# werner-duvaud/muzero-general

Hardware: NVIDIA H100
Metric: self-play env-steps/sec (higher is better)
Workload: dtype f32 nets + f64 tree statistics

## Files before the change

### muzero_general_b200/csrc/fc_search.cu

```cuda
#include "fc_net.cuh"
#include "tree.cuh"
#include "kernels.h"

#include <stdlib.h>
#include <algorithm>
#include <vector>

namespace mz {

struct GameSmem {
    int vsum, mval, root_prior, visit, expansion, reward, prior, path, path_reward, hidden, act, bytes;
};

__host__ __device__ inline GameSmem game_smem_layout(int N, int A, int E, int maxw, bool keep_hidden) {
    GameSmem L;
    const int S = (N + 1) * A;
    const int Epad = (E + 3) & ~3;
    int off = 0;
    auto take = [&](int bytes) { int o = off; off = (off + bytes + 15) & ~15; return o; };
    L.vsum = take(S * 8);
    L.mval = take(S * 8);
    L.root_prior = take(A * 8);
    L.visit = take(S * 4);
    L.expansion = take(S * 4);
    L.reward = take(S * 4);
    L.prior = take(S * 4);
    L.path = take((N + 2) * 4);
    L.path_reward = take((N + 2) * 4);
    L.hidden = take((keep_hidden ? (N + 1) * Epad : 0) * 4);
    L.act = take(9 * maxw * 4);
    off += 16;
    L.bytes = off;
    return L;
}

enum { kPhRoot, kPhSelect, kPhNet, kPhExpand, kPhBackup, kPhLevels, kPhRounds, kPhSims, kPhSums,
       kPhStart = kPhSums, kPhEnd, kPhCount };
#ifdef MZ_FC_PHASES
constexpr int kPhMaxGames = 1 << 16;
__device__ unsigned long long g_fc_phase[kPhMaxGames][kPhCount];
MZ_DEVINL unsigned long long global_ns() {
    unsigned long long t;
    asm volatile("mov.u64 %0, %%globaltimer;" : "=l"(t));
    return t;
}
struct PhaseClock {
    int row = -1;
    unsigned last = 0;
    MZ_DEVINL void start(int g, bool leader) {
        row = (leader && g < kPhMaxGames) ? g : -1;
        if (row >= 0) atomicExch(&g_fc_phase[row][kPhStart], global_ns());
        last = (unsigned)clock();
    }
    MZ_DEVINL void finish() { if (row >= 0) atomicExch(&g_fc_phase[row][kPhEnd], global_ns()); }
    MZ_DEVINL void mark(int p) {
        const unsigned now = (unsigned)clock();
        if (row >= 0) atomicAdd(&g_fc_phase[row][p], (unsigned long long)(now - last));
        last = now;
    }
    MZ_DEVINL void count(int p, int n) { if (row >= 0) atomicAdd(&g_fc_phase[row][p], (unsigned long long)n); }
};
#else
struct PhaseClock {
    MZ_DEVINL void start(int, bool) {}
    MZ_DEVINL void finish() {}
    MZ_DEVINL void mark(int) {}
    MZ_DEVINL void count(int, int) {}
};
#endif

template <typename SH>
constexpr int fixed_actions() {
    if constexpr (SH::kEnabled) return SH::A;
    else return 0;
}

template <int G, bool kTeacher, typename SH, int kP>
__global__ void __launch_bounds__(kFcMaxThreads, 2) fc_search_kernel(const __grid_constant__ FcSearchArgs a) {
    extern __shared__ __align__(16) unsigned char smem[];
    constexpr int kA = fixed_actions<SH>();
    const int N = a.N, A = kA ? kA : a.A;
    double* s_pbc = reinterpret_cast<double*>(smem);
    double* s_sqrt = s_pbc + (N + 2);
    float* s_blob = reinterpret_cast<float*>(s_sqrt + (N + 2));
    for (int i = threadIdx.x; i < N + 2; i += blockDim.x) { s_pbc[i] = a.pbc[i]; s_sqrt[i] = a.sqrtn[i]; }
    if (!kTeacher)
        for (int i = threadIdx.x; i < a.net.blob_floats; i += blockDim.x) s_blob[i] = a.blob[i];
    __syncthreads();

    const int shared_bytes = ((2 * (N + 2) * 8 + (kTeacher ? 0 : a.net.blob_floats) * 4) + 15) & ~15;
    const GameSmem L = game_smem_layout(N, A, a.net.E, a.net.maxw, !kTeacher);
    const int groups_per_cta = blockDim.x / G;
    const int gi = threadIdx.x / G;
    const int lane = LaneGroup<G>::lane();
    unsigned char* mine = smem + shared_bytes + (size_t)gi * L.bytes;

    TreeConst c;
    c.A = A; c.N = N; c.P = a.P; c.discount = a.discount; c.noise_frac = a.noise_frac; c.noise_alpha = a.noise_alpha; c.seed = a.seed;
    c.pbc = s_pbc; c.sqrtn = s_sqrt; c.ucb = a.ucb;

    GameTree t;
    t.vsum = reinterpret_cast<double*>(mine + L.vsum);
    t.mval = reinterpret_cast<double*>(mine + L.mval);
    t.root_prior = reinterpret_cast<double*>(mine + L.root_prior);
    t.visit = reinterpret_cast<int*>(mine + L.visit);
    t.expansion = reinterpret_cast<int*>(mine + L.expansion);
    t.reward = reinterpret_cast<float*>(mine + L.reward);
    t.prior = reinterpret_cast<float*>(mine + L.prior);
    t.path = reinterpret_cast<int*>(mine + L.path);
    t.path_reward = reinterpret_cast<float*>(mine + L.path_reward);
    float* s_hidden = reinterpret_cast<float*>(mine + L.hidden);
    float* s_act = reinterpret_cast<float*>(mine + L.act);
    const int E = a.net.E, F = a.net.F, S = a.net.S, maxw = a.net.maxw;
    const int Epad = (E + 3) & ~3;
    float* s0 = s_act;
    float* s1 = s_act + maxw;
    float* s2 = s_act + 2 * maxw;
    float* const hb[3][2] = {{s_act + 3 * maxw, s_act + 4 * maxw}, {s_act + 5 * maxw, s_act + 6 * maxw},
                             {s_act + 7 * maxw, s_act + 8 * maxw}};
    const bool fused_heads = (a.net.rew.n == a.net.pol.n) && (a.net.pol.n == a.net.val.n);
    constexpr int kMaxD = select_levels_for(kA ? kA : 2, G);
    const SelectLanes sl = select_lanes<G, kA>(A, min(a.select_levels, kMaxD));
    PhaseClock ph;

    const int warp_first = (int)blockIdx.x * groups_per_cta + (int)(threadIdx.x & ~31u) / G;
    for (int g0 = warp_first; g0 < a.n_games; g0 += gridDim.x * groups_per_cta) {
        const int g_own = g0 + gi - (int)(threadIdx.x & ~31u) / G;
        const bool own = g_own < a.n_games;
        const int g = own ? g_own : a.n_games - 1;
        ph.start(g, lane == 0 && own);
        const int64_t game_id = a.game_id ? a.game_id[g] : (int64_t)g;
        const int move = a.move_index ? a.move_index[g] : 0;
        const int to_play0 = a.to_play ? a.to_play[g] : 0;
        const int first_index = a.first_index ? a.first_index[g] : -1;
        unsigned legal = 0;
        for (int k = 0; k < A; ++k) legal |= (a.legal_mask == nullptr || a.legal_mask[(size_t)g * A + k]) ? (1u << k) : 0u;
        t.legal = legal;
        (void)to_play0;

        float root_value, root_reward, logit = 0.0f;
        if (kTeacher) {
            root_value = a.teacher.root_value[g];
            root_reward = a.teacher.root_reward[g];
        } else {
            load_vector<G>(a.obs + (size_t)g * a.net.obs_elems, s1, a.net.obs_elems);
            float* raw = mlp_forward<G>(a.net.rep, s_blob, s1, s0, s1, s2);
            rescale_unit_range<G>(raw, s_hidden, E);
            float* pol = mlp_forward<G>(a.net.pol, s_blob, s_hidden, s0, s1, s2);
            logit = (lane < A) ? pol[lane] : 0.0f;
            LaneGroup<G>::sync();
            float* val = mlp_forward<G>(a.net.val, s_blob, s_hidden, s0, s1, s2);
            root_value = support_to_scalar_group<G>(val, S);
            LaneGroup<G>::sync();
            root_reward = inverse_value_transform(0.0f);
        }
        float prior;
        if (kTeacher) prior = (lane < A) ? a.teacher.root_priors[(size_t)g * A + lane] : 0.0f;
        else prior = group_softmax_masked<G>(logit, lane < A && ((legal >> lane) & 1u));
        if (a.trace.root_priors_raw && lane < A && own) a.trace.root_priors_raw[(size_t)g * A + lane] = ((legal >> lane) & 1u) ? prior : 0.0f;
        if (a.trace.root_reward && lane == 0 && own) a.trace.root_reward[g] = root_reward;
        tree_init_root<G, kA>(c, t, prior, root_reward,
                              (a.add_noise && a.noise) ? a.noise + (size_t)g * A : nullptr, a.add_noise && !a.noise,
                              game_id, move, (a.trace.noise && own) ? a.trace.noise + (size_t)g * A : nullptr);
        ph.mark(kPhRoot);

        int max_depth = 0;
        for (int sim = 0; sim < N; ++sim) {
            int rounds;
            const Leaf leaf = tree_select_lookahead<G, kMaxD, kA>(c, t, sl, sim, game_id, move, first_index, rounds);
            ph.mark(kPhSelect);
            ph.count(kPhLevels, leaf.depth);
            ph.count(kPhRounds, rounds);
            float value, reward;
            if (kTeacher) {
                value = a.teacher.value[(size_t)g * N + sim];
                reward = a.teacher.reward[(size_t)g * N + sim];
                prior = (lane < A) ? a.teacher.priors[((size_t)g * N + sim) * A + lane] : 0.0f;
            } else {
                const float* h = s_hidden + (size_t)leaf.parent_exp * Epad;
                float* hn = s_hidden + (size_t)t.n_expanded * Epad;
                if constexpr (SH::kEnabled) {
                    fc_recurrent_fixed<G, SH>(a.net, s_blob, h, leaf.action, hn, s0, s1, hb[0][0], hb[1][0], hb[2][0], prior, value, reward);
                } else {
                float* raw = mlp_forward<G>(a.net.dyn, s_blob, h, s0, s1, s2, leaf.action);
                if (fused_heads) {
                    rescale_unit_range<G>(raw, hn, E);
                    const MlpDesc* const ds[3] = {&a.net.rew, &a.net.pol, &a.net.val};
                    const float* const xs[3] = {raw, hn, hn};
                    float* outs[3];
                    mlp_forward_multi<G, 3>(ds, s_blob, xs, hb, outs);
                    logit = (lane < A) ? outs[1][lane] : 0.0f;
                    support_to_scalar_group2<G>(outs[2], outs[0], S, value, reward);
                    LaneGroup<G>::sync();
                } else {
                    float* rl = mlp_forward<G>(a.net.rew, s_blob, raw, s0, s1, nullptr);
                    reward = support_to_scalar_group<G>(rl, S);
                    LaneGroup<G>::sync();
                    rescale_unit_range<G>(raw, hn, E);
                    float* pol = mlp_forward<G>(a.net.pol, s_blob, hn, s0, s1, s2);
                    logit = (lane < A) ? pol[lane] : 0.0f;
                    LaneGroup<G>::sync();
                    float* vl = mlp_forward<G>(a.net.val, s_blob, hn, s0, s1, s2);
                    value = support_to_scalar_group<G>(vl, S);
                    LaneGroup<G>::sync();
                }
                }
                if constexpr (!SH::kEnabled) prior = group_softmax_masked<G>(logit, lane < A);
            }
            ph.mark(kPhNet);
            if (a.trace.depth && own) {
                const size_t ti = (size_t)g * N + sim;
                if (lane == 0) { a.trace.depth[ti] = leaf.depth; a.trace.value[ti] = value; a.trace.reward[ti] = reward; }
                if (lane < A) a.trace.priors[ti * A + lane] = prior;
                for (int j = lane; j < leaf.depth && j < a.trace.max_depth; j += G)
                    a.trace.actions[ti * a.trace.max_depth + j] = (uint8_t)(t.path[j + 1] % A);
            }
            tree_expand<G, kA>(c, t, leaf, reward, prior);
            ph.mark(kPhExpand);
            tree_backup<G, kP, true>(c, t, leaf, value);
            ph.mark(kPhBackup);
            max_depth = max(max_depth, leaf.depth);
        }
        ph.count(kPhSims, N);

        if (lane < A && own) {
            const bool ok = (legal >> lane) & 1u;
            if (a.visit_counts) a.visit_counts[(size_t)g * A + lane] = ok ? t.visit[lane] : 0;
            if (a.root_priors) a.root_priors[(size_t)g * A + lane] = t.root_prior[lane];
        }
        if (lane == 0 && own) {
            if (a.root_value) a.root_value[g] = (t.root_visit == 0) ? 0.0 : __ddiv_rn(t.root_vsum, (double)t.root_visit);
            if (a.root_predicted_value) a.root_predicted_value[g] = root_value;
            if (a.max_tree_depth) a.max_tree_depth[g] = max_depth;
            if (a.tie_count) a.tie_count[g] = t.ties;
            if (a.value_range) { a.value_range[2 * g] = t.lo; a.value_range[2 * g + 1] = t.hi; }
        }
        if (a.pool.visit && own) {
            const int slots = (N + 1) * A;
            const size_t pb = (size_t)g * slots;
            for (int s = lane; s < t.n_expanded * A; s += G) {
                a.pool.visit[pb + s] = t.visit[s];
                a.pool.vsum[pb + s] = t.vsum[s];
                a.pool.reward[pb + s] = t.reward[s];
                a.pool.prior[pb + s] = t.prior[s];
                a.pool.expansion[pb + s] = t.expansion[s];
            }
            if (lane < A) a.pool.root_prior[(size_t)g * A + lane] = t.root_prior[lane];
            if (!kTeacher && a.pool.hidden)
                for (int i = lane; i < t.n_expanded * E; i += G)
                    a.pool.hidden[(size_t)g * (N + 1) * E + i] = s_hidden[(i / E) * Epad + (i % E)];
            if (lane == 0) {
                a.pool.root_visit[g] = t.root_visit;
                a.pool.root_vsum[g] = t.root_vsum;
                a.pool.n_expanded[g] = t.n_expanded;
            }
        }
        ph.finish();
        LaneGroup<G>::sync();
    }
    (void)F;
}

static size_t fc_cta_smem(int N, int A, int E, int maxw, int blob_floats, bool teacher, int groups) {
    const GameSmem L = game_smem_layout(N, A, E, maxw, !teacher);
    const size_t shared_bytes = ((2 * (size_t)(N + 2) * 8 + (teacher ? 0 : (size_t)blob_floats) * 4) + 15) & ~(size_t)15;
    return shared_bytes + (size_t)groups * L.bytes;
}

bool fc_search_plan(int N, int A, int E, int maxw, int blob_floats, int G, bool teacher, int n_games, int sm_count,
                    size_t smem_per_sm, size_t smem_reserve, size_t smem_cap, int regs, int threads, FcPlan* plan) {
    if (n_games < 1 || sm_count < 1 || G < 1 || regs < 1 || N < 0 || A < 1 || E < 1 || maxw < 1 || blob_floats < 0) return false;
    bool found = false;
    const std::vector<int> sizes = threads != 0 ? std::vector<int>{threads} : std::vector<int>{64, 128, 256};
    for (int t : sizes) {
        if (t % 32 != 0 || t < G || t > kFcMaxThreads) continue;
        const int groups = t / G;
        const size_t smem = fc_cta_smem(N, A, E, maxw, blob_floats, teacher, groups);
        const int by_smem = smem > smem_cap ? 0 : (int)(smem_per_sm / ((smem + smem_reserve + 127) & ~(size_t)127));
        const int by_regs = (65536 / (((regs * 32) + 255) & ~255)) / (t / 32);
        const int per_sm = std::min(std::min(by_smem, by_regs), std::min(2048 / t, 32));
        if (per_sm >= 1) {
            const int slots = per_sm * groups * sm_count;
            const int passes = (n_games + slots - 1) / slots;
            if (!found || passes < plan->passes) {
                *plan = FcPlan{t, groups, per_sm, slots, passes, smem};
                found = true;
            }
        }
    }
    return found;
}

template <int G, bool T, typename SH, int kP>
static cudaError_t launch_kernel(const FcSearchArgs& a, const FcLaunchInfo& l, cudaStream_t stream) {
    fc_search_kernel<G, T, SH, kP><<<l.grid, l.block, l.smem, stream>>>(a);
    return cudaGetLastError();
}

template <int G, bool T, typename SH, int kP = 0>
static cudaError_t prepare_one(const FcSearchArgs& a, bool one_level, int sm_count, FcLaunchState* st, FcPrepared* p) {
    p->select_levels = one_level ? 1 : select_levels_for(a.A, G);
    auto kern = fc_search_kernel<G, T, SH, kP>;
    const void* fn = reinterpret_cast<const void*>(kern);
    int regs = 0;
    for (const auto& k : st->kernels) if (k.fn == fn) regs = k.regs;
    if (regs == 0) {
        cudaError_t err = cudaFuncSetAttribute(kern, cudaFuncAttributeMaxDynamicSharedMemorySize, (int)st->smem_cap);
        if (err == cudaSuccess) err = cudaFuncSetAttribute(kern, cudaFuncAttributePreferredSharedMemoryCarveout, cudaSharedmemCarveoutMaxShared);
        cudaFuncAttributes fa{};
        if (err == cudaSuccess) err = cudaFuncGetAttributes(&fa, kern);
        if (err != cudaSuccess) return err;
        regs = fa.numRegs;
        st->kernels.push_back({fn, regs});
    }
    FcPlan plan;
    if (!fc_search_plan(a.N, a.A, a.net.E, a.net.maxw, a.net.blob_floats, G, T, a.n_games, sm_count, st->smem_per_sm,
                        st->smem_reserve, st->smem_cap, regs, a.threads, &plan))
        return cudaErrorInvalidConfiguration;
    int per_sm = -1;
    for (const auto& s : st->shapes) if (s.fn == fn && s.threads == plan.threads && s.smem == plan.smem) per_sm = s.ctas_per_sm;
    if (per_sm < 0) {
        cudaError_t err = cudaOccupancyMaxActiveBlocksPerMultiprocessor(&per_sm, kern, plan.threads, plan.smem);
        if (err != cudaSuccess) return err;
        st->shapes.push_back({fn, plan.threads, plan.smem, per_sm});
    }
    per_sm = std::min(per_sm, plan.ctas_per_sm);
    if (per_sm < 1) return cudaErrorInvalidConfiguration;
    const int want = (a.n_games + plan.groups - 1) / plan.groups;
    const int grid = std::min(want, per_sm * sm_count);
    p->launch = launch_kernel<G, T, SH, kP>;
    p->fixed_shape = SH::kEnabled;
    p->info = FcLaunchInfo{grid, plan.threads, per_sm, G, plan.smem};
    return cudaSuccess;
}

using CartPoleShape = FcFixedShape<8, 16, 10, 2>;

static cudaError_t prepare_fc_search(const FcSearchArgs& a, int group, bool teacher, bool generic, bool one_level,
                                     int sm_count, FcLaunchState* st, FcPrepared* p) {
    if (!teacher && !generic && fc_matches_fixed<CartPoleShape>(a.net)) {
        if (group == 16 && a.P == 1) return prepare_one<16, false, CartPoleShape, 1>(a, one_level, sm_count, st, p);
        if (group == 16) return prepare_one<16, false, CartPoleShape>(a, one_level, sm_count, st, p);
        if (group == 32 && a.P == 1) return prepare_one<32, false, CartPoleShape, 1>(a, one_level, sm_count, st, p);
        if (group == 32) return prepare_one<32, false, CartPoleShape>(a, one_level, sm_count, st, p);
    }
#define MZ_CASE(GG)                                                                                     \
    case GG:                                                                                            \
        return teacher ? prepare_one<GG, true, FcGenericShape>(a, one_level, sm_count, st, p)           \
                       : prepare_one<GG, false, FcGenericShape>(a, one_level, sm_count, st, p);
    switch (group) {
        MZ_CASE(4)
        MZ_CASE(8)
        MZ_CASE(16)
        MZ_CASE(32)
    }
#undef MZ_CASE
    return cudaErrorInvalidValue;
}

cudaError_t launch_fc_search(const FcSearchArgs& a_in, int group, bool teacher, int sm_count, FcLaunchState* st,
                             cudaStream_t stream) {
    const char* generic = getenv("MZ_FC_GENERIC");
    const char* levels = getenv("MZ_FC_SELECT_LEVELS");
    FcPreparedKey key{a_in.n_games, group, a_in.threads, teacher, generic && generic[0] == '1',
                      levels && levels[0] == '1' && levels[1] == 0};
    FcPrepared& p = st->prepared;
    if (!p.valid || !(p.key == key)) {
        p.valid = false;
        const cudaError_t err = prepare_fc_search(a_in, group, teacher, key.generic, key.one_level, sm_count, st, &p);
        if (err != cudaSuccess) return err;
        p.key = key;
        p.valid = true;
    }
    FcSearchArgs a = a_in;
    a.select_levels = p.select_levels;
    const cudaError_t err = p.launch(a, p.info, stream);
    if (err == cudaSuccess) {
        st->launched = true;
        st->last = p.info;
    }
    return err;
}

#ifdef MZ_FC_PHASES
extern "C" int mz_fc_phase_counters(unsigned long long* out, int reset) {
    cudaError_t e = cudaDeviceSynchronize();
    void* dev = nullptr;
    if (e == cudaSuccess) e = cudaGetSymbolAddress(&dev, g_fc_phase);
    if (e == cudaSuccess && out) {
        std::vector<unsigned long long> rows((size_t)kPhMaxGames * kPhCount);
        e = cudaMemcpy(rows.data(), dev, rows.size() * 8, cudaMemcpyDeviceToHost);
        for (int p = 0; p < kPhSums; ++p) out[p] = 0;
        for (size_t i = 0; i < rows.size(); ++i) if (i % kPhCount < kPhSums) out[i % kPhCount] += rows[i];
    }
    if (e == cudaSuccess && reset) e = cudaMemset(dev, 0, sizeof(g_fc_phase));
    if (e == cudaSuccess) e = cudaDeviceSynchronize();
    return e == cudaSuccess ? 0 : (int)e;
}

extern "C" int mz_fc_phase_spans(unsigned long long* out, int n) {
    if (!out || n < 0 || n > kPhMaxGames) return (int)cudaErrorInvalidValue;
    std::vector<unsigned long long> rows((size_t)n * kPhCount);
    cudaError_t e = cudaDeviceSynchronize();
    if (e == cudaSuccess) e = cudaMemcpyFromSymbol(rows.data(), g_fc_phase, rows.size() * 8);
    for (int g = 0; e == cudaSuccess && g < n; ++g) {
        out[2 * g] = rows[(size_t)g * kPhCount + kPhStart];
        out[2 * g + 1] = rows[(size_t)g * kPhCount + kPhEnd];
    }
    return e == cudaSuccess ? 0 : (int)e;
}
#endif

}
```

### muzero_general_b200/csrc/tree.cuh

```cuda
#pragma once
#include "common.cuh"

namespace mz {

struct TreeConst {
    int A;
    int N;
    int P;
    double discount;
    double noise_frac;
    double noise_alpha;
    uint64_t seed;
    const double* pbc;
    const double* sqrtn;
    const double* ucb;
};

struct GameTree {
    int* visit;
    double* vsum;
    double* mval;
    float* reward;
    float* prior;
    int* expansion;
    double* root_prior;
    int* path;
    float* path_reward;
    int root_visit;
    double root_vsum;
    float root_reward;
    double lo, hi;
    unsigned legal;
    int n_expanded;
    int ties;
    bool own = true;
};

struct Leaf {
    int depth;
    int parent_exp;
    int action;
    int slot;
};

MZ_DEVINL double value_range_normalize(double v, double lo, double hi) {
    if (hi > lo) {
        const double d = __dsub_rn(v, lo);
        const double q = __ddiv_rn(d == 0.0 ? 1.0 : d, __dsub_rn(hi, lo));
        return d == 0.0 ? 0.0 : q;
    }
    return v;
}

MZ_DEVINL double div_by_count(double s, int n, double y) {
    if (!(fabs(s) >= 0x1p-990 && fabs(s) < INFINITY)) return __ddiv_rn(s, (double)n);
    const double q0 = __dmul_rn(s, y);
    const double r = __fma_rn(-q0, (double)n, s);
    return __fma_rn(r, y, q0);
}

MZ_DEVINL int nth_set_bit(unsigned m, int n) { return (int)__fns(m, 0, n + 1); }

template <int G>
MZ_DEVINL float group_softmax_masked(float logit, bool valid) {
    const float m = group_max_f32<G>(valid ? logit : -INFINITY);
    const float e = valid ? expf(logit - m) : 0.0f;
    const float s = group_sum_f32<G>(e);
    return div_pos_or_zero(e, s);
}

template <int G, int kA = 0>
MZ_DEVINL void tree_init_root(const TreeConst& c, GameTree& t, float prior_f32, float root_reward,
                              const double* noise , bool generate_noise = false,
                              int64_t game_id = 0, int move = 0, double* noise_out = nullptr) {
    const int A = kA ? kA : c.A;
    const int k = LaneGroup<G>::lane();
    const bool legal = (k < A) && ((t.legal >> k) & 1u);
    double nz = 0.0;
    bool have_noise = false;
    if (noise != nullptr) {
        nz = legal ? noise[k] : 0.0;
        have_noise = true;
    } else if (generate_noise) {
        const double gm = legal ? philox_gamma(c.seed, game_id, move, k, c.noise_alpha) : 0.0;
        double sum = gm;
        for (int off = G >> 1; off > 0; off >>= 1) sum += shfl_xor_f64(kWarp, sum, off, G);
        nz = gm / sum;
        have_noise = true;
    }
    if (noise_out && k < A && t.own) noise_out[k] = nz;
    if (k < A && t.own) {
        double p = (double)prior_f32;
        if (legal && have_noise) {
            p = __dadd_rn(__dmul_rn(p, __dsub_rn(1.0, c.noise_frac)), __dmul_rn(nz, c.noise_frac));
        }
        t.root_prior[k] = legal ? p : 0.0;
        t.visit[k] = 0;
        t.vsum[k] = 0.0;
        t.reward[k] = 0.0f;
        t.prior[k] = legal ? prior_f32 : 0.0f;
        t.expansion[k] = -1;
    }
    t.root_visit = 0;
    t.root_vsum = 0.0;
    t.root_reward = root_reward;
    t.lo = INFINITY;
    t.hi = -INFINITY;
    t.n_expanded = 1;
    t.ties = 0;
    LaneGroup<G>::sync();
}

template <int G, bool kPool = false>
MZ_DEVINL Leaf tree_select(const TreeConst& c, GameTree& t, int sim, int64_t game_id, int move, int first_index) {
    const int k = LaneGroup<G>::lane();
    const int width = pow2_ceil(c.A);
    int e = 0;
    int n_parent = t.root_visit;
    int depth = 0;
    Leaf leaf;
    bool done = false;
    if (k == 0 && t.own) { t.path[0] = -1; t.path_reward[0] = t.root_reward; }
    do {
        const int base = e * c.A;
        const bool valid = !done && (k < c.A) && (e != 0 || ((t.legal >> k) & 1u));
        double score = -INFINITY;
        int nc = 0, child_exp_k = -1;
        float reward_k = 0.0f;
        if (valid) {
            nc = t.visit[base + k];
            child_exp_k = t.expansion[base + k];
            const double pr = (e == 0) ? t.root_prior[k] : (double)t.prior[base + k];
            double mv = 0.0, tab_pbc = 0.0, tab_sqrt = 0.0;
            if (kPool) {
                reward_k = t.reward[base + k];
                mv = t.mval[base + k];
                tab_pbc = __ldg(c.pbc + n_parent);
                tab_sqrt = __ldg(c.sqrtn + n_parent);
                if (child_exp_k >= 0) {
                    const int nb = child_exp_k * c.A;
                    prefetch_l1(t.visit + nb); prefetch_l1(t.expansion + nb); prefetch_l1(t.prior + nb);
                    prefetch_l1(t.reward + nb); prefetch_l1(t.mval + nb);
                    prefetch_l1(t.mval + nb + c.A - 1);
                }
            }
            double pbc;
            if (kPool) {
                pbc = __dmul_rn(tab_pbc, __ddiv_rn(tab_sqrt, (double)(nc + 1)));
            } else if (c.ucb) {
                pbc = __ldg(c.ucb + n_parent * (c.N + 2) + nc);
            } else {
                const double q = __ddiv_rn(c.sqrtn[n_parent], (double)(nc + 1));
                pbc = __dmul_rn(c.pbc[n_parent], q);
            }
            score = __dmul_rn(pbc, pr);
            if (nc > 0) {
                if (!kPool) reward_k = t.reward[base + k];
                const double v = value_range_normalize(kPool ? mv : t.mval[base + k], t.lo, t.hi);
                score = __dadd_rn(score, v);
            } else {
                reward_k = 0.0f;
                score = __dadd_rn(score, 0.0);
            }
        }
        const double best = group_max_f64<G>(score, width > G ? G : width);
        const unsigned tied = LaneGroup<G>::ballot(valid && score == best);
        const int n_tied = __popc(tied);
        int pick;
        if (done) {
            pick = 0;
        } else if (n_tied <= 1) {
            pick = max(__ffs(tied) - 1, 0);
        } else {
            int idx;
            if (sim == 0 && depth == 0 && first_index >= 0) {
                idx = first_index < n_tied ? first_index : n_tied - 1;
            } else {
                idx = philox_tie_index(c.seed, game_id, move, sim, depth, n_tied);
                if (!(sim == 0 && depth == 0)) t.ties += 1;
            }
            pick = nth_set_bit(tied, idx);
        }
        const int slot = base + pick;
        const int child_exp = LaneGroup<G>::bcast(child_exp_k, pick);
        const int child_visits = LaneGroup<G>::bcast(nc, pick);
        if (!done) {
            depth += 1;
            if (k == pick && t.own) { t.path[depth] = slot; t.path_reward[depth] = reward_k; }
            if (child_exp < 0) {
                leaf.depth = depth;
                leaf.parent_exp = e;
                leaf.action = pick;
                leaf.slot = slot;
                done = true;
            } else {
                n_parent = child_visits;
                e = child_exp;
            }
        }
    } while (LaneGroup<G>::warp_any(!done));
    LaneGroup<G>::sync();
    return leaf;
}

constexpr int kMaxSelectLevels = 4;

__host__ __device__ constexpr int select_levels_for(int A, int G) {
    int D = 1, lanes = 0, w = 1;
    for (int d = 1; d <= kMaxSelectLevels; ++d) {
        w *= (A < 2 ? 2 : A);
        if (lanes + w > G) break;
        lanes += w;
        D = d;
    }
    return D;
}

struct SelectLanes {
    int D;
    int level;
    int act;
    unsigned walk;
};

template <int G, int kA>
MZ_DEVINL SelectLanes select_lanes(int A_rt, int D) {
    const int A = kA ? kA : A_rt;
    const int k = LaneGroup<G>::lane();
    SelectLanes s{D, 0, 0, 0u};
    int off = 0, w = A, j = 0;
    for (int d = 1; d <= D; ++d) {
        if (k >= off && k < off + w) { s.level = d; j = k - off; }
        off += w;
        w *= A;
    }
    if (s.level > 0) {
        s.act = j % A;
        int q = j / A;
        for (int d = s.level - 1; d >= 1; --d) { s.walk |= (unsigned)(q % A) << (8 * (d - 1)); q /= A; }
    }
    return s;
}

template <int G, int kMaxD, int kA>
MZ_DEVINL Leaf tree_select_lookahead(const TreeConst& c, GameTree& t, const SelectLanes& sl, int sim, int64_t game_id,
                                     int move, int first_index, int& rounds) {
    if (kMaxD <= 1 || sl.D <= 1) {
        const Leaf leaf = tree_select<G>(c, t, sim, game_id, move, first_index);
        rounds = leaf.depth;
        return leaf;
    }
    const int A = kA ? kA : c.A;
    const int D = sl.D;
    const int k = LaneGroup<G>::lane();
    const unsigned seg_mask = (1u << A) - 1u;
    const bool pow2 = (A & (A - 1)) == 0;
    int e = 0;
    int n_parent = t.root_visit;
    int depth = 0;
    Leaf leaf;
    rounds = 0;
    bool done = false;
    if (k == 0 && t.own) { t.path[0] = -1; t.path_reward[0] = t.root_reward; }
    do {
        rounds += done ? 0 : 1;
        int pe = done ? -1 : e, np = n_parent;
#pragma unroll
        for (int d = 1; d < kMaxD; ++d) {
            if (d < sl.level && pe >= 0) {
                const int s = pe * A + (int)((sl.walk >> (8 * (d - 1))) & 0xffu);
                np = t.visit[s];
                pe = t.expansion[s];
            }
        }
        const bool valid = sl.level > 0 && pe >= 0 && (pe != 0 || ((t.legal >> sl.act) & 1u));
        const int slot = pe * A + sl.act;
        double score = -INFINITY;
        int nc = 0, child_exp_k = -1;
        float reward_k = 0.0f;
        if (valid) {
            nc = t.visit[slot];
            child_exp_k = t.expansion[slot];
            const double pr = (pe == 0) ? t.root_prior[sl.act] : (double)t.prior[slot];
            double pbc;
            if (c.ucb) {
                pbc = __ldg(c.ucb + np * (c.N + 2) + nc);
            } else {
                const double q = __ddiv_rn(c.sqrtn[np], (double)(nc + 1));
                pbc = __dmul_rn(c.pbc[np], q);
            }
            score = __dmul_rn(pbc, pr);
            if (nc > 0) {
                reward_k = t.reward[slot];
                score = __dadd_rn(score, value_range_normalize(t.mval[slot], t.lo, t.hi));
            } else {
                score = __dadd_rn(score, 0.0);
            }
        }
        double best = score;
        if (pow2) {
            for (int o = A >> 1; o > 0; o >>= 1) best = fmax(best, shfl_xor_f64(kWarp, best, o, G));
        } else {
            for (int o = 1; o < A; o <<= 1) {
                const int lo = __shfl_down_sync(kWarp, __double2loint(best), o, G);
                const int hi = __shfl_down_sync(kWarp, __double2hiint(best), o, G);
                if (sl.act + o < A) best = fmax(best, __hiloint2double(hi, lo));
            }
            best = shfl_f64(kWarp, best, k - sl.act, G);
        }
        const unsigned tie_bits = LaneGroup<G>::ballot(valid && score == best);
        const unsigned exp_bits = LaneGroup<G>::ballot(valid && child_exp_k >= 0);
        int off = 0, w = A, p = 0, last = 0, pick = 0, dl = 0;
        unsigned picked = 0;
        bool hit_leaf = false;
#pragma unroll
        for (int d = 0; d < kMaxD; ++d) {
            if (d < D && !hit_leaf && !done) {
                const int seg = off + p * A;
                const unsigned tied = (tie_bits >> seg) & seg_mask;
                const int n_tied = __popc(tied);
                const int dd = depth + d;
                if (n_tied <= 1) {
                    pick = max(__ffs(tied) - 1, 0);
                } else {
                    int idx;
                    if (sim == 0 && dd == 0 && first_index >= 0) {
                        idx = first_index < n_tied ? first_index : n_tied - 1;
                    } else {
                        idx = philox_tie_index(c.seed, game_id, move, sim, dd, n_tied);
                        if (!(sim == 0 && dd == 0)) t.ties += 1;
                    }
                    pick = nth_set_bit(tied, idx);
                }
                last = seg + pick;
                picked |= 1u << last;
                dl = d + 1;
                hit_leaf = ((exp_bits >> last) & 1u) == 0;
                off += w;
                w *= A;
                p = p * A + pick;
            }
        }
        if (((picked >> k) & 1u) && t.own) { t.path[depth + sl.level] = slot; t.path_reward[depth + sl.level] = reward_k; }
        const int next = LaneGroup<G>::bcast(hit_leaf ? pe : child_exp_k, last);
        const int next_visits = LaneGroup<G>::bcast(nc, last);
        if (hit_leaf) {
            leaf.depth = depth + dl;
            leaf.parent_exp = next;
            leaf.action = pick;
            leaf.slot = next * A + pick;
            done = true;
        } else if (!done) {
            e = next;
            n_parent = next_visits;
            depth += D;
        }
    } while (LaneGroup<G>::warp_any(!done));
    LaneGroup<G>::sync();
    return leaf;
}

template <int G, int kA = 0>
MZ_DEVINL int tree_expand(const TreeConst& c, GameTree& t, const Leaf& leaf, float reward, float prior_f32) {
    const int A = kA ? kA : c.A;
    const int k = LaneGroup<G>::lane();
    const int e = t.n_expanded;
    if (k == 0 && t.own) {
        t.expansion[leaf.slot] = e;
        t.reward[leaf.slot] = reward;
        t.path_reward[leaf.depth] = reward;
    }
    if (k < A && t.own) {
        const int s = e * A + k;
        t.visit[s] = 0;
        t.vsum[s] = 0.0;
        t.reward[s] = 0.0f;
        t.prior[s] = prior_f32;
        t.expansion[s] = -1;
    }
    t.n_expanded = e + 1;
    LaneGroup<G>::sync();
    return e;
}

template <bool kRcp>
MZ_DEVINL double mean_of(double s, int n) {
    if constexpr (kRcp) return div_by_count(s, n, __drcp_rn((double)n));
    else return __ddiv_rn(s, (double)n);
}

template <int G, int kP = 0, bool kRcp = false>
MZ_DEVINL void tree_backup(const TreeConst& c, GameTree& t, const Leaf& leaf, float leaf_value) {
    const int P = kP ? kP : c.P;
    const int k = LaneGroup<G>::lane();
    const int L = leaf.depth;
    double lo = INFINITY, hi = -INFINITY;
    double v = (double)leaf_value;
    double root_vsum = t.root_vsum;
    const int Lw = G < 32 ? (int)__reduce_max_sync(kWarp, (unsigned)L) : L;
    const bool packed = (Lw < G);
    int my_slot = -1;
    float my_reward = 0.0f;
    if (packed && k <= L) { my_slot = t.path[k]; my_reward = t.path_reward[k]; }
    if (packed) {
        const bool mine = kRcp && k <= L && t.own;
        const int sl = (mine && k > 0) ? my_slot : 0;
        double old_sum = 0.0, y = 1.0;
        int n = 1;
        if constexpr (kRcp) {
            old_sum = k == 0 ? t.root_vsum : t.vsum[sl];
            n = mine ? (k == 0 ? t.root_visit : t.visit[sl]) + 1 : 1;
            y = __drcp_rn((double)n);
        }
        double myv = 0.0;
        for (int j = Lw; j >= 0; --j) {
            const double r = (double)LaneGroup<G>::bcast(my_reward, j);
            const bool same = (P == 1) || (((L - j) & 1) == 0);
            if (j == k) myv = v;
            const double rr = (P == 1) ? r : (same ? -r : r);
            const double vn = __dadd_rn(rr, __dmul_rn(c.discount, v));
            v = j <= L ? vn : v;
        }
        if constexpr (kRcp) {
            const bool same = (P == 1) || (((L - k) & 1) == 0);
            const double add = same ? myv : -myv;
            const double s = __dadd_rn(old_sum, add);
            const double q = div_by_count(mine ? s : 1.0, n, y);
            const double m = __dadd_rn((double)my_reward, __dmul_rn(c.discount, (P == 1) ? q : -q));
            if (mine && k > 0) { t.vsum[sl] = s; t.visit[sl] = n; t.mval[sl] = m; }
            if (mine && k == 0) root_vsum = s;
            lo = mine ? m : lo;
            hi = mine ? m : hi;
        } else if (k <= L && t.own) {
            const bool same = (P == 1) || (((L - k) & 1) == 0);
            const double add = same ? myv : -myv;
            double q;
            if (k == 0) {
                root_vsum = __dadd_rn(t.root_vsum, add);
                q = __ddiv_rn(root_vsum, (double)(t.root_visit + 1));
            } else {
                const double s = __dadd_rn(t.vsum[my_slot], add);
                const int n = t.visit[my_slot] + 1;
                t.vsum[my_slot] = s;
                t.visit[my_slot] = n;
                q = __ddiv_rn(s, (double)n);
            }
            const double m = __dadd_rn((double)my_reward, __dmul_rn(c.discount, (P == 1) ? q : -q));
            if (k > 0) t.mval[my_slot] = m;
            lo = m;
            hi = m;
        }
    } else {
    for (int j = L; j >= 0; --j) {
        const int slot = t.path[j];
        const float rf = t.path_reward[j];
        const double r = (double)rf;
        const bool same = (P == 1) || (((L - j) & 1) == 0);
        if ((j % G) == k && t.own) {
            const double add = same ? v : -v;
            double q;
            if (j == 0) {
                root_vsum = __dadd_rn(t.root_vsum, add);
                q = mean_of<kRcp>(root_vsum, t.root_visit + 1);
            } else {
                const double s = __dadd_rn(t.vsum[slot], add);
                const int n = t.visit[slot] + 1;
                t.vsum[slot] = s;
                t.visit[slot] = n;
                q = mean_of<kRcp>(s, n);
            }
            const double m = __dadd_rn(r, __dmul_rn(c.discount, (P == 1) ? q : -q));
            if (j > 0) t.mval[slot] = m;
            lo = fmin(lo, m);
            hi = fmax(hi, m);
        }
        const double rr = (P == 1) ? r : (same ? -r : r);
        v = __dadd_rn(rr, __dmul_rn(c.discount, v));
    }
    }
    const int width = (Lw + 1 >= G) ? G : pow2_ceil(Lw + 1);
    const unsigned gm = kWarp;
    if (width >= 2) {
        const int half = width >> 1;
        const bool up = (k & half) != 0;
        const double got = shfl_xor_f64(gm, up ? lo : hi, half, G);
        double val = up ? fmax(hi, got) : fmin(lo, got);
        for (int off = half >> 1; off > 0; off >>= 1) {
            const double r = shfl_xor_f64(gm, val, off, G);
            val = up ? fmax(val, r) : fmin(val, r);
        }
        lo = shfl_f64(gm, val, 0, G);
        hi = shfl_f64(gm, val, half, G);
    } else {
        lo = shfl_f64(gm, lo, 0, G);
        hi = shfl_f64(gm, hi, 0, G);
    }
    root_vsum = shfl_f64(gm, root_vsum, 0, G);
    t.root_vsum = root_vsum;
    t.root_visit += 1;
    t.lo = fmin(t.lo, lo);
    t.hi = fmax(t.hi, hi);
    LaneGroup<G>::sync();
}

}
```

Measured before the change: 13.84 million.

## Pack visit/expansion into int2 slots and use reciprocal value normalization

The fused search kernel's tree now stores each slot's child index and visit count as one int2 in shared memory, so selection reads both fields with a single 64-bit load instead of two separate arrays. Value-range normalization during selection computes one reciprocal of (hi-lo) per select call. Each per-child division then becomes a multiply refined with FMA correction steps, kept only when operands lie in a safe range so rounding should stay identical. The cost is a templated tree type, added branching and range checks, and reliance on the correctly rounded reciprocal emulation being exact.

Measured after the change: 14.34 million, median of 6. 3.6% higher.

```diff
diff --git a/muzero_general_b200/csrc/fc_search.cu b/muzero_general_b200/csrc/fc_search.cu
--- a/muzero_general_b200/csrc/fc_search.cu
+++ b/muzero_general_b200/csrc/fc_search.cu
@@ -9,7 +9,7 @@
 namespace mz {
 
 struct GameSmem {
-    int vsum, mval, root_prior, visit, expansion, reward, prior, path, path_reward, hidden, act, bytes;
+    int vsum, mval, root_prior, node, reward, prior, path, path_reward, hidden, act, bytes;
 };
 
 __host__ __device__ inline GameSmem game_smem_layout(int N, int A, int E, int maxw, bool keep_hidden) {
@@ -21,8 +21,7 @@
     L.vsum = take(S * 8);
     L.mval = take(S * 8);
     L.root_prior = take(A * 8);
-    L.visit = take(S * 4);
-    L.expansion = take(S * 4);
+    L.node = take(2 * ((S * 4 + 15) & ~15));
     L.reward = take(S * 4);
     L.prior = take(S * 4);
     L.path = take((N + 2) * 4);
@@ -99,12 +98,11 @@
     c.A = A; c.N = N; c.P = a.P; c.discount = a.discount; c.noise_frac = a.noise_frac; c.noise_alpha = a.noise_alpha; c.seed = a.seed;
     c.pbc = s_pbc; c.sqrtn = s_sqrt; c.ucb = a.ucb;
 
-    GameTree t;
+    PackedGameTree t;
     t.vsum = reinterpret_cast<double*>(mine + L.vsum);
     t.mval = reinterpret_cast<double*>(mine + L.mval);
     t.root_prior = reinterpret_cast<double*>(mine + L.root_prior);
-    t.visit = reinterpret_cast<int*>(mine + L.visit);
-    t.expansion = reinterpret_cast<int*>(mine + L.expansion);
+    t.node = reinterpret_cast<int2*>(mine + L.node);
     t.reward = reinterpret_cast<float*>(mine + L.reward);
     t.prior = reinterpret_cast<float*>(mine + L.prior);
     t.path = reinterpret_cast<int*>(mine + L.path);
@@ -225,7 +223,7 @@
 
         if (lane < A && own) {
             const bool ok = (legal >> lane) & 1u;
-            if (a.visit_counts) a.visit_counts[(size_t)g * A + lane] = ok ? t.visit[lane] : 0;
+            if (a.visit_counts) a.visit_counts[(size_t)g * A + lane] = ok ? t.visits(lane) : 0;
             if (a.root_priors) a.root_priors[(size_t)g * A + lane] = t.root_prior[lane];
         }
         if (lane == 0 && own) {
@@ -239,11 +237,12 @@
             const int slots = (N + 1) * A;
             const size_t pb = (size_t)g * slots;
             for (int s = lane; s < t.n_expanded * A; s += G) {
-                a.pool.visit[pb + s] = t.visit[s];
+                const int2 nd = t.pair(s);
+                a.pool.visit[pb + s] = nd.y;
                 a.pool.vsum[pb + s] = t.vsum[s];
                 a.pool.reward[pb + s] = t.reward[s];
                 a.pool.prior[pb + s] = t.prior[s];
-                a.pool.expansion[pb + s] = t.expansion[s];
+                a.pool.expansion[pb + s] = nd.x;
             }
             if (lane < A) a.pool.root_prior[(size_t)g * A + lane] = t.root_prior[lane];
             if (!kTeacher && a.pool.hidden)
diff --git a/muzero_general_b200/csrc/rn_div.h b/muzero_general_b200/csrc/rn_div.h
--- /dev/null
+++ b/muzero_general_b200/csrc/rn_div.h
@@ -0,0 +1,27 @@
+#pragma once
+#include <math.h>
+
+#ifdef __CUDACC__
+#define MZ_RN_DIV_FN __host__ __device__ __forceinline__
+#else
+#define MZ_RN_DIV_FN static inline
+#endif
+
+#define MZ_RN_DIV_W_MIN 0x1p-500
+#define MZ_RN_DIV_W_MAX 0x1p500
+#define MZ_RN_DIV_D_MIN 0x1p-460
+#define MZ_RN_DIV_D_MAX 0x1p460
+
+MZ_RN_DIV_FN int rn_div_divisor_in_range(double w) { return w >= MZ_RN_DIV_W_MIN && w <= MZ_RN_DIV_W_MAX; }
+MZ_RN_DIV_FN int rn_div_numerator_in_range(double d) {
+    const double a = fabs(d);
+    return a == 0.0 || (a >= MZ_RN_DIV_D_MIN && a <= MZ_RN_DIV_D_MAX);
+}
+
+MZ_RN_DIV_FN double rn_div_by_rcp(double d, double w, double y) {
+    const double q0 = d * y;
+    const double r0 = fma(-q0, w, d);
+    const double q1 = fma(r0, y, q0);
+    const double r1 = fma(-q1, w, d);
+    return fma(r1, y, q1);
+}
diff --git a/muzero_general_b200/csrc/tree.cuh b/muzero_general_b200/csrc/tree.cuh
--- a/muzero_general_b200/csrc/tree.cuh
+++ b/muzero_general_b200/csrc/tree.cuh
@@ -1,5 +1,6 @@
 #pragma once
 #include "common.cuh"
+#include "rn_div.h"
 
 namespace mz {
 
@@ -16,13 +17,30 @@
     const double* ucb;
 };
 
-struct GameTree {
+struct SoaSlots {
     int* visit;
+    int* expansion;
+    MZ_DEVINL int2 pair(int s) const { const int n = visit[s]; return make_int2(expansion[s], n); }
+    MZ_DEVINL int visits(int s) const { return visit[s]; }
+    MZ_DEVINL int child(int s) const { return expansion[s]; }
+    MZ_DEVINL void set_visits(int s, int n) const { visit[s] = n; }
+    MZ_DEVINL void set_child(int s, int e) const { expansion[s] = e; }
+};
+struct PackedSlots {
+    int2* node;
+    MZ_DEVINL int2 pair(int s) const { return node[s]; }
+    MZ_DEVINL int visits(int s) const { return node[s].y; }
+    MZ_DEVINL int child(int s) const { return node[s].x; }
+    MZ_DEVINL void set_visits(int s, int n) const { node[s].y = n; }
+    MZ_DEVINL void set_child(int s, int e) const { node[s].x = e; }
+};
+
+template <class Slots>
+struct GameTreeOf : Slots {
     double* vsum;
     double* mval;
     float* reward;
     float* prior;
-    int* expansion;
     double* root_prior;
     int* path;
     float* path_reward;
@@ -35,6 +53,8 @@
     int ties;
     bool own = true;
 };
+using GameTree = GameTreeOf<SoaSlots>;
+using PackedGameTree = GameTreeOf<PackedSlots>;
 
 struct Leaf {
     int depth;
@@ -43,13 +63,20 @@
     int slot;
 };
 
-MZ_DEVINL double value_range_normalize(double v, double lo, double hi) {
+template <bool kRcp = false>
+MZ_DEVINL double value_range_normalize(double v, double lo, double hi, double y = 0.0) {
     if (hi > lo) {
         const double d = __dsub_rn(v, lo);
+        if (kRcp && y != 0.0 && rn_div_numerator_in_range(d)) return rn_div_by_rcp(d, __dsub_rn(hi, lo), y);
         const double q = __ddiv_rn(d == 0.0 ? 1.0 : d, __dsub_rn(hi, lo));
         return d == 0.0 ? 0.0 : q;
     }
     return v;
+}
+
+MZ_DEVINL double value_range_rcp(double lo, double hi) {
+    const double w = __dsub_rn(hi, lo);
+    return (hi > lo && rn_div_divisor_in_range(w)) ? __drcp_rn(w) : 0.0;
 }
 
 MZ_DEVINL double div_by_count(double s, int n, double y) {
@@ -69,8 +96,8 @@
     return div_pos_or_zero(e, s);
 }
 
-template <int G, int kA = 0>
-MZ_DEVINL void tree_init_root(const TreeConst& c, GameTree& t, float prior_f32, float root_reward,
+template <int G, int kA = 0, class Tree>
+MZ_DEVINL void tree_init_root(const TreeConst& c, Tree& t, float prior_f32, float root_reward,
                               const double* noise , bool generate_noise = false,
                               int64_t game_id = 0, int move = 0, double* noise_out = nullptr) {
     const int A = kA ? kA : c.A;
@@ -95,11 +122,11 @@
             p = __dadd_rn(__dmul_rn(p, __dsub_rn(1.0, c.noise_frac)), __dmul_rn(nz, c.noise_frac));
         }
         t.root_prior[k] = legal ? p : 0.0;
-        t.visit[k] = 0;
+        t.set_visits(k, 0);
         t.vsum[k] = 0.0;
         t.reward[k] = 0.0f;
         t.prior[k] = legal ? prior_f32 : 0.0f;
-        t.expansion[k] = -1;
+        t.set_child(k, -1);
     }
     t.root_visit = 0;
     t.root_vsum = 0.0;
@@ -111,9 +138,10 @@
     LaneGroup<G>::sync();
 }
 
-template <int G, bool kPool = false>
-MZ_DEVINL Leaf tree_select(const TreeConst& c, GameTree& t, int sim, int64_t game_id, int move, int first_index) {
+template <int G, bool kPool = false, bool kRcp = false, class Tree>
+MZ_DEVINL Leaf tree_select(const TreeConst& c, Tree& t, int sim, int64_t game_id, int move, int first_index) {
     const int k = LaneGroup<G>::lane();
+    const double y = kRcp ? value_range_rcp(t.lo, t.hi) : 0.0;
     const int width = pow2_ceil(c.A);
     int e = 0;
     int n_parent = t.root_visit;
@@ -128,11 +156,12 @@
         int nc = 0, child_exp_k = -1;
         float reward_k = 0.0f;
         if (valid) {
-            nc = t.visit[base + k];
-            child_exp_k = t.expansion[base + k];
+            const int2 nd = t.pair(base + k);
+            nc = nd.y;
+            child_exp_k = nd.x;
             const double pr = (e == 0) ? t.root_prior[k] : (double)t.prior[base + k];
             double mv = 0.0, tab_pbc = 0.0, tab_sqrt = 0.0;
-            if (kPool) {
+            if constexpr (kPool) {
                 reward_k = t.reward[base + k];
                 mv = t.mval[base + k];
                 tab_pbc = __ldg(c.pbc + n_parent);
@@ -156,7 +185,7 @@
             score = __dmul_rn(pbc, pr);
             if (nc > 0) {
                 if (!kPool) reward_k = t.reward[base + k];
-                const double v = value_range_normalize(kPool ? mv : t.mval[base + k], t.lo, t.hi);
+                const double v = value_range_normalize<kRcp>(kPool ? mv : t.mval[base + k], t.lo, t.hi, y);
                 score = __dadd_rn(score, v);
             } else {
                 reward_k = 0.0f;
@@ -242,11 +271,11 @@
     return s;
 }
 
-template <int G, int kMaxD, int kA>
-MZ_DEVINL Leaf tree_select_lookahead(const TreeConst& c, GameTree& t, const SelectLanes& sl, int sim, int64_t game_id,
+template <int G, int kMaxD, int kA, class Tree>
+MZ_DEVINL Leaf tree_select_lookahead(const TreeConst& c, Tree& t, const SelectLanes& sl, int sim, int64_t game_id,
                                      int move, int first_index, int& rounds) {
     if (kMaxD <= 1 || sl.D <= 1) {
-        const Leaf leaf = tree_select<G>(c, t, sim, game_id, move, first_index);
+        const Leaf leaf = tree_select<G, false, true>(c, t, sim, game_id, move, first_index);
         rounds = leaf.depth;
         return leaf;
     }
@@ -255,6 +284,7 @@
     const int k = LaneGroup<G>::lane();
     const unsigned seg_mask = (1u << A) - 1u;
     const bool pow2 = (A & (A - 1)) == 0;
+    const double y = value_range_rcp(t.lo, t.hi);
     int e = 0;
     int n_parent = t.root_visit;
     int depth = 0;
@@ -269,8 +299,9 @@
         for (int d = 1; d < kMaxD; ++d) {
             if (d < sl.level && pe >= 0) {
                 const int s = pe * A + (int)((sl.walk >> (8 * (d - 1))) & 0xffu);
-                np = t.visit[s];
-                pe = t.expansion[s];
+                const int2 nd = t.pair(s);
+                np = nd.y;
+                pe = nd.x;
             }
         }
         const bool valid = sl.level > 0 && pe >= 0 && (pe != 0 || ((t.legal >> sl.act) & 1u));
@@ -279,8 +310,9 @@
         int nc = 0, child_exp_k = -1;
         float reward_k = 0.0f;
         if (valid) {
-            nc = t.visit[slot];
-            child_exp_k = t.expansion[slot];
+            const int2 nd = t.pair(slot);
+            nc = nd.y;
+            child_exp_k = nd.x;
             const double pr = (pe == 0) ? t.root_prior[sl.act] : (double)t.prior[slot];
             double pbc;
             if (c.ucb) {
@@ -292,7 +324,7 @@
             score = __dmul_rn(pbc, pr);
             if (nc > 0) {
                 reward_k = t.reward[slot];
-                score = __dadd_rn(score, value_range_normalize(t.mval[slot], t.lo, t.hi));
+                score = __dadd_rn(score, value_range_normalize<true>(t.mval[slot], t.lo, t.hi, y));
             } else {
                 score = __dadd_rn(score, 0.0);
             }
@@ -360,23 +392,23 @@
     return leaf;
 }
 
-template <int G, int kA = 0>
-MZ_DEVINL int tree_expand(const TreeConst& c, GameTree& t, const Leaf& leaf, float reward, float prior_f32) {
+template <int G, int kA = 0, class Tree>
+MZ_DEVINL int tree_expand(const TreeConst& c, Tree& t, const Leaf& leaf, float reward, float prior_f32) {
     const int A = kA ? kA : c.A;
     const int k = LaneGroup<G>::lane();
     const int e = t.n_expanded;
     if (k == 0 && t.own) {
-        t.expansion[leaf.slot] = e;
+        t.set_child(leaf.slot, e);
         t.reward[leaf.slot] = reward;
         t.path_reward[leaf.depth] = reward;
     }
     if (k < A && t.own) {
         const int s = e * A + k;
-        t.visit[s] = 0;
+        t.set_visits(s, 0);
         t.vsum[s] = 0.0;
         t.reward[s] = 0.0f;
         t.prior[s] = prior_f32;
-        t.expansion[s] = -1;
+        t.set_child(s, -1);
     }
     t.n_expanded = e + 1;
     LaneGroup<G>::sync();
@@ -389,8 +421,8 @@
     else return __ddiv_rn(s, (double)n);
 }
 
-template <int G, int kP = 0, bool kRcp = false>
-MZ_DEVINL void tree_backup(const TreeConst& c, GameTree& t, const Leaf& leaf, float leaf_value) {
+template <int G, int kP = 0, bool kRcp = false, class Tree>
+MZ_DEVINL void tree_backup(const TreeConst& c, Tree& t, const Leaf& leaf, float leaf_value) {
     const int P = kP ? kP : c.P;
     const int k = LaneGroup<G>::lane();
     const int L = leaf.depth;
@@ -409,7 +441,7 @@
         int n = 1;
         if constexpr (kRcp) {
             old_sum = k == 0 ? t.root_vsum : t.vsum[sl];
-            n = mine ? (k == 0 ? t.root_visit : t.visit[sl]) + 1 : 1;
+            n = mine ? (k == 0 ? t.root_visit : t.visits(sl)) + 1 : 1;
             y = __drcp_rn((double)n);
         }
         double myv = 0.0;
@@ -427,7 +459,7 @@
             const double s = __dadd_rn(old_sum, add);
             const double q = div_by_count(mine ? s : 1.0, n, y);
             const double m = __dadd_rn((double)my_reward, __dmul_rn(c.discount, (P == 1) ? q : -q));
-            if (mine && k > 0) { t.vsum[sl] = s; t.visit[sl] = n; t.mval[sl] = m; }
+            if (mine && k > 0) { t.vsum[sl] = s; t.set_visits(sl, n); t.mval[sl] = m; }
             if (mine && k == 0) root_vsum = s;
             lo = mine ? m : lo;
             hi = mine ? m : hi;
@@ -440,9 +472,9 @@
                 q = __ddiv_rn(root_vsum, (double)(t.root_visit + 1));
             } else {
                 const double s = __dadd_rn(t.vsum[my_slot], add);
-                const int n = t.visit[my_slot] + 1;
+                const int n = t.visits(my_slot) + 1;
                 t.vsum[my_slot] = s;
-                t.visit[my_slot] = n;
+                t.set_visits(my_slot, n);
                 q = __ddiv_rn(s, (double)n);
             }
             const double m = __dadd_rn((double)my_reward, __dmul_rn(c.discount, (P == 1) ? q : -q));
@@ -464,9 +496,9 @@
                 q = mean_of<kRcp>(root_vsum, t.root_visit + 1);
             } else {
                 const double s = __dadd_rn(t.vsum[slot], add);
-                const int n = t.visit[slot] + 1;
+                const int n = t.visits(slot) + 1;
                 t.vsum[slot] = s;
-                t.visit[slot] = n;
+                t.set_visits(slot, n);
                 q = mean_of<kRcp>(s, n);
             }
             const double m = __dadd_rn(r, __dmul_rn(c.discount, (P == 1) ? q : -q));
```
